# pennucci/PulsePortraiture

Hardware: AMD Instinct MI355X
Metric: subint_fits_per_sec (higher is better)
Workload: dtype f64

## Files before the change

pulseportraiture_amd/csrc/pp_fftq.h:

```cpp
#pragma once
#include "pp_fft.h"

namespace pp {

__device__ __forceinline__ void lane_swap32(double& a, double& b) {
    unsigned alo = (unsigned)__double2loint(a), ahi = (unsigned)__double2hiint(a);
    unsigned blo = (unsigned)__double2loint(b), bhi = (unsigned)__double2hiint(b);
    auto r0 = __builtin_amdgcn_permlane32_swap(alo, blo, false, false);
    auto r1 = __builtin_amdgcn_permlane32_swap(ahi, bhi, false, false);
    a = __hiloint2double((int)r1[0], (int)r0[0]);
    b = __hiloint2double((int)r1[1], (int)r0[1]);
}
__device__ __forceinline__ void lane_swap16(double& a, double& b) {
    unsigned alo = (unsigned)__double2loint(a), ahi = (unsigned)__double2hiint(a);
    unsigned blo = (unsigned)__double2loint(b), bhi = (unsigned)__double2hiint(b);
    auto r0 = __builtin_amdgcn_permlane16_swap(alo, blo, false, false);
    auto r1 = __builtin_amdgcn_permlane16_swap(ahi, bhi, false, false);
    a = __hiloint2double((int)r1[0], (int)r0[0]);
    b = __hiloint2double((int)r1[1], (int)r0[1]);
}

__device__ __forceinline__ int fftq_lambda(int t) { return 4 * (t >> 4) + (t & 3) + 16 * ((t >> 2) & 3); }
__device__ __forceinline__ int fftq_lane_of(int lam) { return 16 * ((lam >> 2) & 3) + (lam & 3) + 4 * ((lam >> 4) & 3); }

constexpr int FFTQ_LDS_ELEMS = 4 * 272;

template <int WHEN = 0, typename T1, typename T2, typename Mid>
__device__ __forceinline__ void fftq1024_from(cplx (&v)[16], cplx* lds, T1 get_t1, T2 get_t2, int tid,
                                              double* power, Mid mid) {
    dft16_first(v);
    if (WHEN == 0) mid();
    const cplx t1 = get_t1();
    dft16_second(v);
    {
        cplx wq[16];
        wq[1] = t1;
#pragma unroll
        for (int j = 2; j < 16; ++j) {
            if (j % 2 == 0) {
                const cplx h = wq[j / 2];
                wq[j] = make_double2(fma(h.x, h.x, -h.y * h.y), 2.0 * h.x * h.y);
            } else wq[j] = cmul(wq[j - 1], wq[1]);
        }
#pragma unroll
        for (int j = 1; j < 16; ++j) v[j] = cmul(v[j], wq[j]);
    }
    if (WHEN == 1) mid();
    const cplx t2 = get_t2();
#pragma unroll
    for (int j = 0; j < 8; ++j) {
        lane_swap32(v[j].x, v[j + 8].x);
        lane_swap32(v[j].y, v[j + 8].y);
    }
#pragma unroll
    for (int j = 0; j < 16; ++j) {
        if (j & 4) continue;
        lane_swap16(v[j].x, v[j + 4].x);
        lane_swap16(v[j].y, v[j + 4].y);
    }
    if (WHEN == 2) mid();
    dft16_first(v);
    {
        const cplx w2 = make_double2(fma(t2.x, t2.x, -t2.y * t2.y), 2.0 * t2.x * t2.y);
        const cplx w3 = cmul(w2, t2);
#pragma unroll
        for (int c = 0; c < 4; ++c) {
            v[4 + c] = cmul(v[4 + c], t2);
            v[8 + c] = cmul(v[8 + c], w2);
            v[12 + c] = cmul(v[12 + c], w3);
        }
    }
    {
        cplx* wbase = lds + (tid >> 4) * 272 + 17 * (tid & 15);
#pragma unroll
        for (int j = 0; j < 16; ++j) wbase[j] = v[j];
        lds_sync<64>();
        const cplx* rbase = lds + (tid >> 4) * 272 + (tid & 15);
#pragma unroll
        for (int j = 0; j < 16; ++j) v[j] = rbase[17 * j];
        lds_sync<64>();
    }
    if (WHEN == 3) mid();
    dft_reg<16>(v);
    if (power) {
        double acc = 0.0;
#pragma unroll
        for (int j = 0; j < 16; ++j) {
            if (j == 0 && tid == 0) { const double dM = v[0].x - v[0].y; acc += dM * dM; }
            else acc += cnorm(v[j]);
        }
        *power += acc;
    }
}

template <int WHEN = 0, typename Mid>
__device__ __forceinline__ void fftq1024(cplx (&v)[16], cplx* lds, const cplx t1, const cplx t2, int tid,
                                         double* power, Mid mid) {
    fftq1024_from<WHEN>(v, lds, [&]() { return t1; }, [&]() { return t2; }, tid, power, mid);
}

__device__ __forceinline__ int fftq512_lambda(int t) {
    return 4 * ((t >> 5) & 1) + 2 * ((t >> 4) & 1) + 32 * ((t >> 3) & 1) + 16 * ((t >> 2) & 1) + 8 * ((t >> 1) & 1) + (t & 1);
}
__device__ __forceinline__ int fftq512_lane_of(int lam) {
    return 32 * ((lam >> 2) & 1) + 16 * ((lam >> 1) & 1) + 8 * ((lam >> 5) & 1) + 4 * ((lam >> 4) & 1) + 2 * ((lam >> 3) & 1) + (lam & 1);
}
constexpr int FFTQ512_LDS_ELEMS = 8 * 72;

__device__ __forceinline__ double lane_xor8(double v) {
    int lo = __double2loint(v), hi = __double2hiint(v);
    lo = __builtin_amdgcn_update_dpp(lo, lo, 0x128, 0xF, 0xF, false);
    hi = __builtin_amdgcn_update_dpp(hi, hi, 0x128, 0xF, 0xF, false);
    return __hiloint2double(hi, lo);
}

template <int WHEN = 0, typename Mid>
__device__ __forceinline__ void fftq512(cplx (&v)[8], cplx* lds, const cplx t1, const cplx t2, const cplx t3, int tid,
                                        double* power, Mid mid) {
    dft_reg<8>(v);
    if (WHEN == 0) mid();
    {
        cplx wq[8];
        wq[1] = t1;
#pragma unroll
        for (int j = 2; j < 8; ++j) {
            if (j % 2 == 0) {
                const cplx h = wq[j / 2];
                wq[j] = make_double2(fma(h.x, h.x, -h.y * h.y), 2.0 * h.x * h.y);
            } else wq[j] = cmul(wq[j - 1], wq[1]);
        }
#pragma unroll
        for (int j = 1; j < 8; ++j) v[j] = cmul(v[j], wq[j]);
    }
#pragma unroll
    for (int j = 0; j < 4; ++j) {
        lane_swap32(v[j].x, v[j + 4].x);
        lane_swap32(v[j].y, v[j + 4].y);
    }
#pragma unroll
    for (int j = 0; j < 8; ++j) {
        if (j & 2) continue;
        lane_swap16(v[j].x, v[j + 2].x);
        lane_swap16(v[j].y, v[j + 2].y);
    }
    dft4(v[0], v[2], v[4], v[6]);
    dft4(v[1], v[3], v[5], v[7]);
    {
        const cplx w2 = make_double2(fma(t2.x, t2.x, -t2.y * t2.y), 2.0 * t2.x * t2.y);
        const cplx w3 = cmul(w2, t2);
#pragma unroll
        for (int c = 0; c < 2; ++c) {
            v[2 + c] = cmul(v[2 + c], t2);
            v[4 + c] = cmul(v[4 + c], w2);
            v[6 + c] = cmul(v[6 + c], w3);
        }
    }
    {
        const bool up = (tid & 8) != 0;
        const double sg = up ? -1.0 : 1.0;
        const cplx w = up ? t3 : make_double2(1.0, 0.0);
#pragma unroll
        for (int j = 0; j < 8; ++j) {
            const cplx p = make_double2(lane_xor8(v[j].x), lane_xor8(v[j].y));
            const cplx d = make_double2(fma(sg, v[j].x, p.x), fma(sg, v[j].y, p.y));
            v[j] = cmul(d, w);
        }
    }
    {
        cplx* wbase = lds + (tid >> 3) * 72 + 9 * (tid & 7);
#pragma unroll
        for (int j = 0; j < 8; ++j) wbase[j] = v[j];
        lds_sync<64>();
        const cplx* rbase = lds + (tid >> 3) * 72 + (tid & 7);
#pragma unroll
        for (int j = 0; j < 8; ++j) v[j] = rbase[9 * j];
        lds_sync<64>();
    }
    if (WHEN == 3) mid();
    dft_reg<8>(v);
    if (power) {
        double acc = 0.0;
#pragma unroll
        for (int j = 0; j < 8; ++j) {
            if (j == 0 && tid == 0) { const double dM = v[0].x - v[0].y; acc += dM * dM; }
            else acc += cnorm(v[j]);
        }
        *power += acc;
    }
}

template <int M> struct FftQ;
template <> struct FftQ<1024> {
    static constexpr int R = 16, LDS_ELEMS = FFTQ_LDS_ELEMS;
    static __device__ __forceinline__ int lambda(int t) { return fftq_lambda(t); }
    static __device__ __forceinline__ int lane_of(int lam) { return fftq_lane_of(lam); }
    template <int WHEN, typename Mid>
    static __device__ __forceinline__ void run(cplx (&v)[16], cplx* lds, const cplx* twB, int tid, double* power, Mid mid) {
        const cplx t1 = twB[2 * tid], t2 = twB[32 * (tid & 15)];
        fftq1024<WHEN>(v, lds, t1, t2, tid, power, mid);
    }
};
template <> struct FftQ<512> {
    static constexpr int R = 8, LDS_ELEMS = FFTQ512_LDS_ELEMS;
    static __device__ __forceinline__ int lambda(int t) { return fftq512_lambda(t); }
    static __device__ __forceinline__ int lane_of(int lam) { return fftq512_lane_of(lam); }
    template <int WHEN, typename Mid>
    static __device__ __forceinline__ void run(cplx (&v)[8], cplx* lds, const cplx* twB, int tid, double* power, Mid mid) {
        const cplx t1 = twB[2 * tid], t2 = twB[16 * (tid & 15)], t3 = twB[64 * (tid & 7)];
        fftq512<WHEN>(v, lds, t1, t2, t3, tid, power, mid);
    }
};


__device__ __forceinline__ cplx split_pair(const cplx zk, cplx zc, const cplx wb) {
    zc.y = -zc.y;
    const cplx E = make_double2(zk.x + zc.x, zk.y + zc.y);
    const cplx O = make_double2(zk.x - zc.x, zk.y - zc.y);
    const cplx wo = cmul(wb, O);
    return make_double2(E.x + wo.y, E.y - wo.x);
}

template <int N>
__device__ __forceinline__ void taylor_terms(const bool first, double (&tm)[N], const cplx x, const cplx z, const double kap) {
    static_assert(PP_TJ == 10 && N >= PP_TSTRIDE, "power ladder written for order 10");
    const double p2 = kap * kap, p4 = p2 * p2, p6 = p4 * p2, p8 = p4 * p4, p10 = p8 * p2;
    const double ui = z.y * kap;
    const double ax = fabs(x.x) + fabs(x.y);
    if (first) {
        tm[0] = z.x;
        tm[1] = ui;
        tm[2] = p2 * z.x;
        tm[3] = p2 * ui;
        tm[4] = p4 * z.x;
        tm[5] = p4 * ui;
        tm[6] = p6 * z.x;
        tm[7] = p6 * ui;
        tm[8] = p8 * z.x;
        tm[9] = p8 * ui;
        tm[10] = p10 * z.x;
        tm[11] = (p10 * kap) * ax;
    } else {
        tm[0] += z.x;
        tm[1] += ui;
        tm[2] = fma(p2, z.x, tm[2]);
        tm[3] = fma(p2, ui, tm[3]);
        tm[4] = fma(p4, z.x, tm[4]);
        tm[5] = fma(p4, ui, tm[5]);
        tm[6] = fma(p6, z.x, tm[6]);
        tm[7] = fma(p6, ui, tm[7]);
        tm[8] = fma(p8, z.x, tm[8]);
        tm[9] = fma(p8, ui, tm[9]);
        tm[10] = fma(p10, z.x, tm[10]);
        tm[11] = fma(p10 * kap, ax, tm[11]);
    }
}

template <typename Raw, int R>
__device__ __forceinline__ void load_row_pieces(Raw (&cur)[1][R], const void* nxrow, const int tid, const int k0, const int k1) {
    const char* gb = reinterpret_cast<const char*>(nxrow);
    const unsigned boff = (unsigned)tid * (unsigned)sizeof(Raw);
#pragma unroll
    for (int k = 0; k < R; ++k)
        if (k >= k0 && k < k1) cur[0][k] = load_row_once<Raw>(gb + (size_t)(k * 64) * sizeof(Raw) + boff);
}

}
```

pulseportraiture_amd/csrc/pp_xspec1024q.h:

```cpp
#pragma once
#include "pp_fftq.h"


namespace pp {

constexpr unsigned PP_TICKET_WINDOW_NUM = 3u, PP_TICKET_WINDOW_DEN = 4u;
__device__ __forceinline__ int ticket_moment(const long long nrows) {
    const unsigned share = (unsigned)(nrows / (long long)gridDim.x) + 1u;
    return 1 + (int)(((blockIdx.x * 2654435761u) >> 8) % (share * PP_TICKET_WINDOW_NUM / PP_TICKET_WINDOW_DEN + 1u));
}

template <int M, typename Tin>
__device__ __forceinline__ const Tin* next_row_of(const XspecArgs& a, const unsigned more_nx, const int i_nx, const int n_nx,
                                                  const size_t rc) {
    const size_t rn = more_nx ? (size_t)sub_of(a.act, i_nx) * a.nchan_full + (a.coff + n_nx * a.cstep) : rc;
    return reinterpret_cast<const Tin*>(a.data) + rn * (2 * M);
}

constexpr int FFTQ_FREE_ELEM0 = 3 * 272 + 16, FFTQ_FREE_PITCH = 17;

template <int M, bool TAIL, bool ONE = true>
__device__ __forceinline__ void store_row_results(const XspecArgs& a, const size_t rc, const int tid, double tv) {
    constexpr int H = M + 1, kc = (int)(0.75 * H);
  if constexpr (ONE) {
    const int q = wave_reduce16_index(tid);
    const double th = 0.5 * tv;
    double val = (q <= PP_TJ && ((q & 3) == 1 || (q & 3) == 2)) ? -th : th;
    double* dst = a.tay + tay_idx(rc, q < PP_TSTRIDE ? q : 0);
    if (q >= PP_TSTRIDE) { val = tv; dst = a.sdraw + rc; }
    if (TAIL) {
        const double nz = sqrt(tv / (2.0 * M) / (double)(H - kc));
        if (q > PP_TSTRIDE) { val = nz; dst = a.noise + rc; }
    }
    typedef double __attribute__((address_space(1)))* gdp_t;
    *(gdp_t)(uintptr_t)dst = val;
  } else {
    if ((tid & 3) == 0) {
        const int q = wave_reduce16_index(tid);
        if (q < PP_TSTRIDE) {
            tv *= 0.5;
            a.tay[tay_idx(rc, q)] = (q <= PP_TJ && ((q & 3) == 1 || (q & 3) == 2)) ? -tv : tv;
        }
    }
    if (tid == 4 * PP_TSTRIDE) a.sdraw[rc] = tv;
    if (TAIL && tid == 4 * (PP_TSTRIDE + 1)) a.noise[rc] = sqrt(tv / (2.0 * M) / (double)(H - kc));
  }
}

__device__ __forceinline__ void first_row_landed() { __builtin_amdgcn_s_waitcnt(0x0F70); }

constexpr int Q_PREFETCH_F64 = 1, Q_PREFETCH_F32 = 0;
template <typename Tin, bool TAIL>
__global__ __launch_bounds__(64, 2) void k_xspec_q1024(XspecArgs a) {
    constexpr int M = 1024, T = 64, R1 = 16, PER1 = 1;
    constexpr int NSL = 7;
    typedef typename RawOf<Tin>::type Raw;
    constexpr int NRED = PP_TSTRIDE + (TAIL ? 2 : 1);
    static_assert(NRED <= 16, "wave_reduce_lds takes 16 values");
    constexpr int WRED = PP_WRED_DOUBLES(NRED) / 2;
    constexpr int LDSN = WRED > FFTQ_LDS_ELEMS ? WRED : FFTQ_LDS_ELEMS;
    static_assert(2 * LDSN >= PP_TAIL_LDS_DOUBLES, "tail_work's layout of this kernel's LDS");
    constexpr bool F64 = sizeof(Tin) == 8;
    constexpr int NML = (F64 && TAIL) ? 2 : 0;
    constexpr bool TWL = F64 && !TAIL, TWR = F64 && TAIL;
    constexpr bool ROWTOP = !TAIL;
    constexpr int NTW = TWL ? 2 : 0;
    __shared__ cplx lds[LDSN + 64 * (NML + NTW)];
    static_assert(sizeof(lds) <= 19456, "eight workgroups per CU");
    static_assert(FFTQ_FREE_ELEM0 + 15 * FFTQ_FREE_PITCH < FFTQ_LDS_ELEMS && FFTQ_FREE_ELEM0 >= 64 * (TAIL ? 12 : 7) &&
                  2 * FFTQ_FREE_ELEM0 >= PP_WRED_DOUBLES(NRED), "t2's elements are outside everything a row writes");
    cplx* const ldsm = lds + LDSN + threadIdx.x;
    int tid = threadIdx.x;
    const long long nrows = (long long)a.nsub * a.nchan;
    Raw cur[PER1][R1];
    cplx t1 = a.twB[2 * tid], t2 = a.twB[32 * (tid & 15)];
    const int lam0 = fftq_lambda(tid);
    cplx wb0 = a.twB[lam0 ? lam0 : 64];
    const cplx wbT = a.twB[64];
    cplx* const ldt2 = lds + FFTQ_FREE_ELEM0;
    cplx* const ldtw = lds + LDSN + 64 * NML;
    auto put_lane_consts = [&](const cplx p1, const cplx p2, const cplx pb) {
        if (!TWL) return;
        ldt2[FFTQ_FREE_PITCH * (tid & 15)] = p2;
        ldtw[tid] = p1;
        ldtw[64 + tid] = pb;
        lds_sync<T>();
    };
    put_lane_consts(t1, t2, wb0);
    int tail_after = 0x7fffffff;
    if (a.tail) tail_after = ticket_moment(nrows);
    RowWalk<true> rw;
    rw.start(nrows, a.mwords, a.ticket, a.ticket_base);
    long long row = rw.row;
    int n = 0, i = 0;
    if (rw.more) {
        n = __builtin_amdgcn_readfirstlane((int)(row / a.nsub));
        i = __builtin_amdgcn_readfirstlane((int)(row % a.nsub));
        const size_t rc = (size_t)sub_of(a.act, i) * a.nchan_full + (a.coff + n * a.cstep);
        stage_load_global<M, T, R1>(cur, reinterpret_cast<const Tin*>(a.data) + rc * (2 * M), tid);
    }
    cplx mv2[NSL];
    const cplx* mheld = nullptr;
    const cplx* mrow = nullptr;
    int n_held = -1, ktn = 0;
    int i_nx = i, n_nx = n;
    if (ROWTOP) first_row_landed();
#pragma unroll 1
    for (int phase = 0; phase < 2; ++phase) {
    if (phase == 1) {
        if (!a.tail) break;
        tail_work(a.tail, reinterpret_cast<double*>(lds), 2 * (LDSN + 64 * NML), tid, 1);
        tail_after = 0x7fffffff;
        if (TWL) {
            const int lamr = fftq_lambda(tid);
            put_lane_consts(as_global(a.twB)[2 * tid], as_global(a.twB)[32 * (tid & 15)], as_global(a.twB)[lamr ? lamr : 64]);
        }
    }
    for (; rw.more && tail_after != 0; rw.advance(), row = rw.row, i = i_nx, n = n_nx, --tail_after) {
        rw.draw(a.ticket);
        rw.peek(nrows, a.ticket_base, a.mwords);
        asm volatile("" : "+v"(tid));
        const int lam = fftq_lambda(tid);
        const bool l0 = (lam == 0);
        const int kb = l0 ? 64 : lam;
        if (TWR) {
            t1 = as_global(a.twB)[2 * tid];
            t2 = as_global(a.twB)[32 * (tid & 15)];
            wb0 = as_global(a.twB)[kb];
        } else if (!TWL) {
            asm volatile("" : "+v"(t1.x), "+v"(t1.y), "+v"(t2.x), "+v"(t2.y), "+v"(wb0.x), "+v"(wb0.y));
        }
        const int ia = sub_of(a.act, i), ne = a.coff + n * a.cstep;
        const size_t rc = (size_t)ia * a.nchan_full + ne;
        if (channel_lookup(a, ia, n, ne, M, n_held, mrow, ktn) && mrow != mheld) {
#pragma unroll
            for (int j = 0; j < NSL; ++j) {
                const cplx mval = mrow[kb + 64 * j - 1];
                if (j < NSL - NML) mv2[j] = mval; else ldsm[64 * (j - (NSL - NML))] = mval;
            }
            mheld = mrow;
        }
        const double phin = ROWTOP ? load_uniform(a.ph0 + rc) : a.ph0[rc];
        double sd = 0.0;
        cplx v[R1];
#pragma unroll
        for (int k = 0; k < R1; ++k) v[k] = to_cplx(cur[0][k]);
        constexpr bool HALVES = F64;
        const Tin* nxrow = nullptr;
        auto load_some = [&](int k0, int k1) { load_row_pieces<Raw>(cur, nxrow, tid, k0, k1); };
        rw.next(i, n, i_nx, n_nx, nrows, a.nsub, a.ticket_base, a.ticket, a.mwords);
        nxrow = next_row_of<M, Tin>(a, rw.more_nx, i_nx, n_nx, rc);
        auto prefetch = [&]() {
            __builtin_amdgcn_sched_barrier(0);
            load_some(0, HALVES ? R1 / 2 : R1);
            __builtin_amdgcn_sched_barrier(0);
        };
        fftq1024_from<(sizeof(Tin) == 8 ? Q_PREFETCH_F64 : Q_PREFETCH_F32)>(
            v, lds, [&]() { return NTW ? ldtw[tid] : t1; }, [&]() { return TWL ? ldt2[FFTQ_FREE_PITCH * (tid & 15)] : t2; },
            tid, &sd, prefetch);
        __builtin_amdgcn_sched_barrier(0);
        {
            cplx* pub = lds + tid;
#pragma unroll
            for (int r = 0; r < NSL; ++r) pub[64 * r] = v[9 + r];
            if (TAIL) {
#pragma unroll
                for (int r = 0; r < 5; ++r) pub[64 * (NSL + r)] = v[r];
            }
            lds_sync<T>();
        }
        if (NTW) wb0 = ldtw[64 + tid];
        double tail = 0.0;
        if (TAIL) {
            const double h = 0.70710678118654752440;
            const cplx* pt = lds + fftq_lane_of((64 - lam) & 63) + (l0 ? 64 : 0);
            cplx wt = l0 ? make_double2(-h, -h) : cmul(wb0, make_double2(-h, -h));
#pragma unroll
            for (int kd = 12; kd < 16; ++kd) {
                tail += cnorm(split_pair(v[kd], pt[64 * (NSL + 15 - kd)], wt));
                wt = cmul(wt, wbT);
            }
            tail *= 0.25;
            if (tid == 0) { const double dM = v[0].x - v[0].y; tail += dM * dM; }
        }
        if (HALVES) {
            __builtin_amdgcn_sched_barrier(0);
            load_some(R1 / 2, R1);
            __builtin_amdgcn_sched_barrier(0);
        }
        const cplx* pc = lds + fftq_lane_of((64 - lam) & 63);
        const cplx el = unit_phasor<true>((double)kb, phin);
        const cplx wst = make_double2(bcast_lane0(el.x), bcast_lane0(el.y));
        cplx e = el, wb = wb0;
        const int ktu = __builtin_amdgcn_readfirstlane(ktn);
        const double kap0 = PP_TWO_PI * (double)kb;
        double tm[PP_TSTRIDE];
        cplx zc_nx = pc[64 * 6];
#pragma unroll
        for (int j = 0; j < NSL; ++j) {
            if (j > 0 && !(64 * j < ktu)) break;
            const cplx zc = zc_nx;
            if (j + 1 < NSL && 64 * (j + 1) < ktu) zc_nx = pc[64 * (5 - j)];
            if (j == 0 || 64 * j < ktu) {
                const cplx dd = split_pair(csel(l0, v[j + 1], v[j]), zc, wb);
                const cplx mj = (j < NSL - NML) ? mv2[j < NSL - NML ? j : 0] : ldsm[64 * (j - (NSL - NML))];
                const cplx x = cmulc(dd, mj);
                const cplx z = cmul(x, e);
                const double kap = j == 0 ? kap0 : kap0 + kconst<true>(PP_TWO_PI * (double)(64 * j));
                taylor_terms(j == 0, tm, x, z, kap);
            }
            if (j + 1 < NSL && 64 * (j + 1) < ktu) {
                wb = cmul(wb, wbT);
                e = cmul(e, wst);
            }
        }
        double tr[NRED];
#pragma unroll
        for (int j = 0; j < PP_TSTRIDE; ++j) tr[j] = tm[j];
        tr[PP_TSTRIDE] = sd;
        if (TAIL) tr[NRED - 1] = tail;
        lds_sync<T>();
        double tv = wave_reduce_lds(tr, tid, reinterpret_cast<double*>(lds));
        store_row_results<M, TAIL, ROWTOP>(a, rc, tid, tv);
        lds_sync<T>();
    }
    }
    if (a.tail) tail_work(a.tail, reinterpret_cast<double*>(lds), 2 * (LDSN + 64 * NML), tid, 1 << 30);
}


constexpr int PP_QF512_WPS = 3;
template <int M, typename Tin, bool TAIL>
__global__ __launch_bounds__(64, (M == 1024 ? 2 : PP_QF512_WPS)) void k_xspec_qf(XspecArgs a) {
    typedef FftQ<M> Q;
    constexpr int T = 64, R1 = Q::R, PER1 = 1;
    constexpr int NSL = R1;
    constexpr int JT = (3 * NSL) / 4;
    static_assert((int)(0.75 * (M + 1)) == 64 * JT, "the noise tail starts on a slot boundary");
    typedef typename RawOf<Tin>::type Raw;
    constexpr int NRED = PP_TSTRIDE + (TAIL ? 2 : 1);
    constexpr int WRED = PP_WRED_DOUBLES(NRED) / 2;
    constexpr int LDSN0 = Q::LDS_ELEMS > 64 * NSL ? Q::LDS_ELEMS : 64 * NSL;
    constexpr int LDSN = WRED > LDSN0 ? WRED : LDSN0;
    static_assert(M != 1024 || 2 * LDSN >= PP_TAIL_LDS_DOUBLES, "tail_work's layout of this kernel's LDS");
    __shared__ cplx lds[LDSN];
    int tid = threadIdx.x;
    constexpr bool QTOP = M == 1024 && !TAIL;
    const long long nrows = (long long)a.nsub * a.nchan;
    Raw cur[PER1][R1];
    const cplx wbT = a.twB[64];
    int tail_after = 0x7fffffff;
    if (M == 1024 && a.tail) tail_after = ticket_moment(nrows);
    RowWalk<true> rw;
    rw.start(nrows, a.mwords, a.ticket, a.ticket_base);
    long long row = rw.row;
    int n = 0, i = 0;
    if (rw.more) {
        n = __builtin_amdgcn_readfirstlane((int)(row / a.nsub));
        i = __builtin_amdgcn_readfirstlane((int)(row % a.nsub));
        const size_t rc = (size_t)sub_of(a.act, i) * a.nchan_full + (a.coff + n * a.cstep);
        stage_load_global<M, T, R1>(cur, reinterpret_cast<const Tin*>(a.data) + rc * (2 * M), tid);
    }
    int i_nx = i, n_nx = n;
    const cplx* mrow = nullptr;
    int n_held = -1, ktn = 0;
    constexpr bool MHOLD = M == 512;
    cplx mv[NSL];
    const cplx* mheld = nullptr;
    if (QTOP) first_row_landed();
#pragma unroll 1
    for (int phase = 0; phase < 2; ++phase) {
    if (phase == 1) {
        if (!(M == 1024 && a.tail)) break;
        tail_work(a.tail, reinterpret_cast<double*>(lds), 2 * LDSN, tid, 1);
        tail_after = 0x7fffffff;
    }
    for (; rw.more && tail_after != 0; rw.advance(), row = rw.row, i = i_nx, n = n_nx, --tail_after) {
        rw.draw(a.ticket);
        rw.peek(nrows, a.ticket_base, a.mwords);
        asm volatile("" : "+v"(tid));
        const int lam = Q::lambda(tid);
        const bool l0 = (lam == 0);
        const int kb = l0 ? 64 : lam;
        const cplx wb0 = as_global(a.twB)[kb];
        const int ia = sub_of(a.act, i), ne = a.coff + n * a.cstep;
        const size_t rc = (size_t)ia * a.nchan_full + ne;
        const bool looked = channel_lookup(a, ia, n, ne, M, n_held, mrow, ktn);
        if (MHOLD && looked && mrow != mheld) {
#pragma unroll
            for (int j = 0; j < NSL; ++j) mv[j] = mrow[kb + 64 * j - 1];
            mheld = mrow;
        }
        const double phin = QTOP ? load_uniform(a.ph0 + rc) : a.ph0[rc];
        double sd = 0.0;
        cplx v[R1];
#pragma unroll
        for (int k = 0; k < R1; ++k) v[k] = to_cplx(cur[0][k]);
        auto template_loads = [&]() {
            if (MHOLD) return;
            __builtin_amdgcn_sched_barrier(0);
#pragma unroll
            for (int j = 0; j < NSL; ++j) mv[j] = mrow[kb + 64 * j - 1];
            __builtin_amdgcn_sched_barrier(0);
        };
        Q::template run<3>(v, lds, as_global(a.twB), tid, &sd, template_loads);
        __builtin_amdgcn_sched_barrier(0);
        {
            cplx* pub = lds + tid;
#pragma unroll
            for (int s = 0; s < NSL; ++s) pub[64 * s] = v[s];
            lds_sync<T>();
        }
        const Tin* nxrow;
        auto load_some = [&](int k0, int k1) { load_row_pieces<Raw>(cur, nxrow, tid, k0, k1); };
        {
            __builtin_amdgcn_sched_barrier(0);
            rw.next(i, n, i_nx, n_nx, nrows, a.nsub, a.ticket_base, a.ticket, a.mwords);
            nxrow = next_row_of<M, Tin>(a, rw.more_nx, i_nx, n_nx, rc);
            load_some(0, R1 / 2);
            __builtin_amdgcn_sched_barrier(0);
        }
        const cplx* pc = lds + Q::lane_of((64 - lam) & 63);
        const cplx el = unit_phasor<true>((double)kb, phin);
        const cplx wst = make_double2(bcast_lane0(el.x), bcast_lane0(el.y));
        cplx e = el, wb = wb0;
        const int ktu = __builtin_amdgcn_readfirstlane(ktn);
        const double kap0 = PP_TWO_PI * (double)kb;
        double tm[PP_TSTRIDE];
        double tail = 0.0;
        cplx zc_nx = pc[64 * (NSL - 1)];
#pragma unroll
        for (int j = 0; j < NSL; ++j) {
            if (!TAIL && j > NSL / 2 && !(64 * j < ktu)) break;
            const cplx zc = zc_nx;
            if (j + 1 < NSL && (TAIL || 64 * (j + 1) < ktu)) zc_nx = pc[64 * (NSL - 2 - j)];
            if (j == NSL / 2) {
                __builtin_amdgcn_sched_barrier(0);
                load_some(R1 / 2, R1);
                __builtin_amdgcn_sched_barrier(0);
            }
            const bool keep = (j == 0 || 64 * j < ktu);
            if (keep || (TAIL && j >= JT - 1)) {
                const cplx dd = split_pair(csel(l0, v[(j + 1) & (NSL - 1)], v[j]), zc, wb);
                if (TAIL && j >= JT - 1) {
                    const double pw = cnorm(dd);
                    tail += (j >= JT || l0) ? pw : 0.0;
                }
              if (keep) {
                const cplx x = cmulc(dd, mv[j]);
                const cplx z = cmul(x, e);
                const double kap = j == 0 ? kap0 : kap0 + kconst<true>(PP_TWO_PI * (double)(64 * j));
                taylor_terms(j == 0, tm, x, z, kap);
              }
            }
            if (TAIL || (j + 1 < NSL && 64 * (j + 1) < ktu)) {
                wb = cmul(wb, wbT);
                e = cmul(e, wst);
            }
        }
        double tr[NRED];
#pragma unroll
        for (int j = 0; j < PP_TSTRIDE; ++j) tr[j] = tm[j];
        tr[PP_TSTRIDE] = sd;
        if (TAIL) tr[NRED - 1] = 0.25 * tail;
        lds_sync<T>();
        double tv = wave_reduce_lds(tr, tid, reinterpret_cast<double*>(lds));
        store_row_results<M, TAIL, QTOP>(a, rc, tid, tv);
        lds_sync<T>();
    }
    }
    if (M == 1024 && a.tail) tail_work(a.tail, reinterpret_cast<double*>(lds), 2 * LDSN, tid, 1 << 30);
}

}
```

Baseline: 72240.

## Fast-path consecutive subint rows within a claimed chunk and group row loads

When the TWL variant is active, the row loop detects a freshly claimed, fully-owned chunk of consecutive subints and, for the remaining rows, advances the row index, bitmask and next-row pointer arithmetically. This skips the ticket draw/peek, sub_of lookup, channel_lookup and rw.next on those rows. Prefetch loads of the next row are also regrouped around a mid-span scalar base pointer, so each load uses a small signed immediate offset instead of separate address math. The cost is more branching and bookkeeping state, and the fast path relies on the conditions being checked correctly (no active mask, no slot, no mwords).

```diff
diff --git a/pulseportraiture_amd/csrc/pp_fftq.h b/pulseportraiture_amd/csrc/pp_fftq.h
--- a/pulseportraiture_amd/csrc/pp_fftq.h
+++ b/pulseportraiture_amd/csrc/pp_fftq.h
@@ -255,13 +255,27 @@
     }
 }
 
-template <typename Raw, int R>
+template <typename Raw, int R, bool MID = false>
 __device__ __forceinline__ void load_row_pieces(Raw (&cur)[1][R], const void* nxrow, const int tid, const int k0, const int k1) {
     const char* gb = reinterpret_cast<const char*>(nxrow);
     const unsigned boff = (unsigned)tid * (unsigned)sizeof(Raw);
-#pragma unroll
-    for (int k = 0; k < R; ++k)
-        if (k >= k0 && k < k1) cur[0][k] = load_row_once<Raw>(gb + (size_t)(k * 64) * sizeof(Raw) + boff);
-}
-
-}
+    if constexpr (MID) {
+        constexpr int PIECE = 64 * (int)sizeof(Raw), SPAN = 8192, PER = SPAN / PIECE;
+#pragma unroll
+        for (int g = 0; g * PER < R; ++g) {
+            if (!(g * PER < k1 && (g + 1) * PER > k0)) continue;
+            const char* mid = gb + (g * SPAN + SPAN / 2);
+            asm volatile("" : "+s"(mid));
+            mid = as_global(mid);
+#pragma unroll
+            for (int k = g * PER; k < (g + 1) * PER && k < R; ++k)
+                if (k >= k0 && k < k1) cur[0][k] = load_row_once<Raw>(mid + (ptrdiff_t)(k * PIECE - g * SPAN - SPAN / 2) + boff);
+        }
+    } else {
+#pragma unroll
+        for (int k = 0; k < R; ++k)
+            if (k >= k0 && k < k1) cur[0][k] = load_row_once<Raw>(gb + (size_t)(k * 64) * sizeof(Raw) + boff);
+    }
+}
+
+}
diff --git a/pulseportraiture_amd/csrc/pp_xspec1024q.h b/pulseportraiture_amd/csrc/pp_xspec1024q.h
--- a/pulseportraiture_amd/csrc/pp_xspec1024q.h
+++ b/pulseportraiture_amd/csrc/pp_xspec1024q.h
@@ -104,6 +104,7 @@
     const cplx* mrow = nullptr;
     int n_held = -1, ktn = 0;
     int i_nx = i, n_nx = n;
+    constexpr bool FASTROW = TWL;
     if (ROWTOP) first_row_landed();
 #pragma unroll 1
     for (int phase = 0; phase < 2; ++phase) {
@@ -116,9 +117,13 @@
             put_lane_consts(as_global(a.twB)[2 * tid], as_global(a.twB)[32 * (tid & 15)], as_global(a.twB)[lamr ? lamr : 64]);
         }
     }
+    unsigned fast_left = 0u;
+    size_t rc_prev = 0;
     for (; rw.more && tail_after != 0; rw.advance(), row = rw.row, i = i_nx, n = n_nx, --tail_after) {
-        rw.draw(a.ticket);
-        rw.peek(nrows, a.ticket_base, a.mwords);
+        if (!FASTROW) {
+            rw.draw(a.ticket);
+            rw.peek(nrows, a.ticket_base, a.mwords);
+        }
         asm volatile("" : "+v"(tid));
         const int lam = fftq_lambda(tid);
         const bool l0 = (lam == 0);
@@ -130,26 +135,51 @@
         } else if (!TWL) {
             asm volatile("" : "+v"(t1.x), "+v"(t1.y), "+v"(t2.x), "+v"(t2.y), "+v"(wb0.x), "+v"(wb0.y));
         }
-        const int ia = sub_of(a.act, i), ne = a.coff + n * a.cstep;
-        const size_t rc = (size_t)ia * a.nchan_full + ne;
-        if (channel_lookup(a, ia, n, ne, M, n_held, mrow, ktn) && mrow != mheld) {
-#pragma unroll
-            for (int j = 0; j < NSL; ++j) {
-                const cplx mval = mrow[kb + 64 * j - 1];
-                if (j < NSL - NML) mv2[j] = mval; else ldsm[64 * (j - (NSL - NML))] = mval;
-            }
-            mheld = mrow;
-        }
+        size_t rc;
+        const Tin* nxrow = nullptr;
+        if (FASTROW && fast_left != 0u) {
+            --fast_left;
+            rc = rc_prev + (size_t)(unsigned)a.nchan_full;
+            rw.row_nx = rw.row + 1u;
+            rw.bits &= rw.bits - 1u;
+            i_nx = i + 1;
+            nxrow = reinterpret_cast<const Tin*>(a.data) + (rc + (size_t)(unsigned)a.nchan_full) * (2 * M);
+        } else {
+            if (FASTROW) {
+                rw.draw(a.ticket);
+                rw.peek(nrows, a.ticket_base, a.mwords);
+            }
+            const int ia = sub_of(a.act, i), ne = a.coff + n * a.cstep;
+            rc = (size_t)ia * a.nchan_full + ne;
+            if (channel_lookup(a, ia, n, ne, M, n_held, mrow, ktn) && mrow != mheld) {
+#pragma unroll
+                for (int j = 0; j < NSL; ++j) {
+                    const cplx mval = mrow[kb + 64 * j - 1];
+                    if (j < NSL - NML) mv2[j] = mval; else ldsm[64 * (j - (NSL - NML))] = mval;
+                }
+                mheld = mrow;
+            }
+            if (FASTROW) {
+                const bool first_of_chunk = rw.fresh != 0u;
+                rw.next(i, n, i_nx, n_nx, nrows, a.nsub, a.ticket_base, a.ticket, a.mwords);
+                nxrow = next_row_of<M, Tin>(a, rw.more_nx, i_nx, n_nx, rc);
+                const bool whole = first_of_chunk && rw.bits == 0xfffffffcu && i + (PP_ROW_CHUNK - 1) < a.nsub &&
+                                   !a.mwords && !a.act && !a.slot;
+                fast_left = (unsigned)__builtin_amdgcn_readfirstlane(whole ? PP_ROW_CHUNK - 2 : 0);
+            }
+        }
+        rc_prev = rc;
         const double phin = ROWTOP ? load_uniform(a.ph0 + rc) : a.ph0[rc];
         double sd = 0.0;
         cplx v[R1];
 #pragma unroll
         for (int k = 0; k < R1; ++k) v[k] = to_cplx(cur[0][k]);
         constexpr bool HALVES = F64;
-        const Tin* nxrow = nullptr;
-        auto load_some = [&](int k0, int k1) { load_row_pieces<Raw>(cur, nxrow, tid, k0, k1); };
-        rw.next(i, n, i_nx, n_nx, nrows, a.nsub, a.ticket_base, a.ticket, a.mwords);
-        nxrow = next_row_of<M, Tin>(a, rw.more_nx, i_nx, n_nx, rc);
+        auto load_some = [&](int k0, int k1) { load_row_pieces<Raw, R1, FASTROW>(cur, nxrow, tid, k0, k1); };
+        if (!FASTROW) {
+            rw.next(i, n, i_nx, n_nx, nrows, a.nsub, a.ticket_base, a.ticket, a.mwords);
+            nxrow = next_row_of<M, Tin>(a, rw.more_nx, i_nx, n_nx, rc);
+        }
         auto prefetch = [&]() {
             __builtin_amdgcn_sched_barrier(0);
             load_some(0, HALVES ? R1 / 2 : R1);
```

Result: faster. 73140, median of 6 (+1.2%).
